# namada-net/masp

Hardware: AMD Instinct MI355X
Metric: Spend proofs/sec (higher is better)
Workload: dtype u32; 1 GPU; BASELINE.json configs[3]: batch of 256 distinct Spend proofs per step on one MI355X (throughput mode); proofs_per_gpu=4352, distinct_witnesses_per_gpu=256, ntt_log2=17, batch_cap=256, slots=4, calls_in_flight=4, hw_queues=4, parallelism=proofs sharded over 1 GPU(s), no data-path collective, gather of the proofs

## Files before the change

masp_amd/csrc/internal.h:

```cpp
#pragma once
#include <hip/hip_runtime.h>

#include <algorithm>
#include <array>
#include <condition_variable>
#include <cstring>
#include <deque>
#include <map>
#include <memory>
#include <mutex>
#include <shared_mutex>
#include <string>
#include <thread>
#include <vector>

#include "device/io.hpp"
#include "device/ntt_geom.h"
#include "launch.h"
#include "msm_host.h"
#include <atomic>
#include "util.h"

namespace masp {

template <class T>
struct DevBuf {
    T* p = nullptr;
    size_t cap = 0;
    ~DevBuf() { release(); }
    void release() {
        if (p) dev_free(p);
        p = nullptr;
        cap = 0;
    }
    int reserve(size_t n) {
        if (n <= cap) return MASP_HIP_OK;
        release();
        HIP_TRY(dev_malloc(&p, sizeof(T) * std::max<size_t>(n, 1)));
        cap = n;
        return MASP_HIP_OK;
    }
    int upload(const T* h, size_t n, hipStream_t s) {
        int rc = reserve(n);
        if (rc) return rc;
        if (n) HIP_TRY(hipMemcpyAsync(p, h, sizeof(T) * n, hipMemcpyHostToDevice, s));
        return MASP_HIP_OK;
    }
};

static inline Fr fr_from_u64_mont(uint64_t x) {
    Fr v = fe_zero<FrCfg>();
    v.v[0] = (uint32_t)x;
    v.v[1] = (uint32_t)(x >> 32);
    return fe_to_mont(v);
}
static inline Fr fr_const(const uint32_t* limbs) {
    Fr v;
    for (int i = 0; i < 8; ++i) v.v[i] = limbs[i];
    return v;
}

struct NttDomain {
    uint32_t logm = 0;
    size_t m = 0;
    DevBuf<Fr> tw_fwd, tw_inv, coset_scale, h_scale;
    Fr c_scale;
    int init(uint32_t logm_, hipStream_t s) {
        logm = logm_;
        m = (size_t)1 << logm;
        Fr omega = fr_const(FrCfg::ROOT_OF_UNITY);
        for (uint32_t i = logm; i < 32; ++i) omega = fe_sqr(omega);
        Fr omega_inv = fe_inv(omega);
        Fr minv = fe_inv(fr_from_u64_mont(m));
        Fr g = fr_const(FrCfg::GEN), ginv = fr_const(FrCfg::GEN_INV);
        uint32_t e[2] = {(uint32_t)m, (uint32_t)((uint64_t)m >> 32)};
        const Fr zinv = fe_inv(fe_sub(fe_pow(g, e, 2), fe_one<FrCfg>()));
        const Fr mzinv = fe_mul(minv, zinv);
        c_scale = fe_from_mont(mzinv);
        Fr one = fe_one<FrCfg>();
        size_t half = std::max<size_t>(m / 2, 1);
        int rc;
        if ((rc = tw_fwd.reserve(half)) || (rc = tw_inv.reserve(half)) || (rc = coset_scale.reserve(m)) || (rc = h_scale.reserve(m))) return rc;
        launch_fr_powers(s, tw_fwd.p, (uint32_t)half, omega, one, 0);
        launch_fr_powers(s, tw_inv.p, (uint32_t)half, omega_inv, one, 0);
        launch_fr_powers(s, coset_scale.p, (uint32_t)m, g, minv, 0);
        launch_fr_powers(s, h_scale.p, (uint32_t)m, ginv, mzinv, 1);
        HIP_TRY(hipStreamSynchronize(s));
        return MASP_HIP_OK;
    }
    void passes(hipStream_t s, Fr* data, const Fr* tw, uint32_t np = 1) const {
        for (uint32_t s0 = 0; s0 < logm;) {
            uint32_t nst = std::min<uint32_t>(NTT_LT, logm - s0);
            launch_ntt_pass(s, data, tw, logm, s0, nst, np);
            s0 += nst;
        }
    }
};

struct Circuit {
    uint32_t n_inputs = 0, n_aux = 0, n_constraints = 0, nrows = 0, logm = 0;
    size_t m = 0;
    DevBuf<uint32_t> rowptr[3], col[3];
    DevBuf<uint32_t> row_order[3];
    uint32_t n_long_rows[3] = {0, 0, 0};
    DevBuf<Fr> coef[3];
    DevBuf<uint32_t> a_var, b_var;
    uint32_t na = 0, nbq = 0;
    DevBuf<VkDevice> vk;
    DevBuf<G1Xyzz> fb1;
    DevBuf<G2Xyzz> fb2;
    BasesG1 h, l, a, b1;
    BasesG1 hl;
    BasesG2 b2;
    BasesG2 b2_lone;
    bool g1_endo = false;
    NttDomain* dom = nullptr;
};

struct Slot {
    hipStream_t stream = nullptr;
    hipEvent_t done = nullptr;
    MsmWorkspace<FpOps> ws1;
    MsmWorkspace<Fp2Ops> ws2;
    static constexpr int N_AUX = 4;
    hipStream_t aux[N_AUX] = {nullptr, nullptr, nullptr, nullptr};
    hipEvent_t ev_fork = nullptr, ev_sort_b = nullptr, ev_fixed = nullptr, ev_join[N_AUX] = {nullptr, nullptr, nullptr, nullptr};
    hipEvent_t ev_uploaded = nullptr;
    MsmWorkspace<FpOps> ws_l, ws_a, ws_b;
    DevBuf<Fr> w, inp, abc, wm, ev[3], x0, x1, h, hl, sa, sb;
    DevBuf<G1Xyzz> res1, asm1;
    DevBuf<G2Xyzz> res2, asm2;
    DevBuf<uint32_t> rs;
    DevBuf<uint8_t> proof;
    DevBuf<int> flags;
    MsmProfile prof;
    bool profiling = false;
    static constexpr int N_LONE_MARKS = 12;
    hipEvent_t ev_lone[N_LONE_MARKS] = {};
    bool lone_marked = false;
    void lone_mark(hipStream_t st, int id) {
        if (!profiling) return;
        if (!ev_lone[id] && hipEventCreate(&ev_lone[id]) != hipSuccess) return;
        (void)hipEventRecord(ev_lone[id], st);
        if (id == N_LONE_MARKS - 1) lone_marked = true;
    }
    uint32_t ntt_sub = 8;
    uint8_t* h_stage = nullptr;
    size_t h_stage_cap = 0;
    uint8_t* h_proof = nullptr;
    size_t h_proof_cap = 0;
    int* h_flags = nullptr;
    struct LoneGraph {
        const void *circuit, *w, *abc, *rs, *proof;
        size_t w_stride;
        uint32_t np;
        bool mont;
        int runs;
        bool dead;
        hipGraphExec_t exec;
    };
    std::vector<LoneGraph> graphs;
    uint64_t graph_epoch = 0;
    bool lone_graph = false;
    std::atomic<uint64_t> graph_launches{0};
    void drop_graphs() {
        for (auto& g : graphs)
            if (g.exec) hipGraphExecDestroy(g.exec);
        graphs.clear();
    }
    ~Slot() {
        drop_graphs();
        if (done) hipEventDestroy(done);
        for (hipEvent_t e : ev_join)
            if (e) hipEventDestroy(e);
        for (hipEvent_t e : ev_lone)
            if (e) hipEventDestroy(e);
        if (ev_fork) hipEventDestroy(ev_fork);
        if (ev_uploaded) hipEventDestroy(ev_uploaded);
        if (ev_sort_b) hipEventDestroy(ev_sort_b);
        if (ev_fixed) hipEventDestroy(ev_fixed);
        if (h_stage) hipHostFree(h_stage);
        if (h_proof) hipHostFree(h_proof);
        if (h_flags) hipHostFree(h_flags);
    }
    void configure(const masp_hip_options& o) {
        ntt_sub = (uint32_t)o.ntt_sub_batch;
        ws1.tree_levels = o.bucket_tree_levels;
        ws2.tree_levels = o.bucket_tree_levels_g2;
        ws1.tree_levels_shared = o.bucket_tree_levels_g2;
        ws1.tree_sub = ws2.tree_sub = (uint32_t)o.bucket_tree_sub_batch;
        ws2.tree.arena = &ws1.tree.own;
        ws1.tree.own.limit = (size_t)o.bucket_tree_scratch_mb << 20;
        lone_graph = o.lone_proof_graph > 0;
    }
    int init(const std::array<hipStream_t, 5>& streams) {
        stream = streams[0];
        for (int i = 0; i < N_AUX; ++i) aux[i] = streams[1 + i];
        HIP_TRY(hipEventCreateWithFlags(&done, hipEventDisableTiming));
        HIP_TRY(hipEventCreateWithFlags(&ev_fork, hipEventDisableTiming));
        HIP_TRY(hipEventCreateWithFlags(&ev_uploaded, hipEventDisableTiming));
        HIP_TRY(hipEventCreateWithFlags(&ev_sort_b, hipEventDisableTiming));
        HIP_TRY(hipEventCreateWithFlags(&ev_fixed, hipEventDisableTiming));
        for (hipEvent_t& e : ev_join) HIP_TRY(hipEventCreateWithFlags(&e, hipEventDisableTiming));
        HIP_TRY(hipHostMalloc(&h_flags, sizeof(int)));
        int rc;
        if ((rc = flags.reserve(1))) return rc;
        return reserve_batch(1);
    }
    int reserve_batch(size_t np) {
        int rc;
        if ((rc = res1.reserve(4 * np)) || (rc = res2.reserve(np)) || (rc = asm1.reserve(6 * np)) || (rc = asm2.reserve(np)) || (rc = rs.reserve(16 * np)) || (rc = proof.reserve(192 * np))) return rc;
        if (np > h_proof_cap) {
            if (h_proof) hipHostFree(h_proof);
            h_proof = nullptr;
            HIP_TRY(hipHostMalloc(&h_proof, 192 * np));
            h_proof_cap = np;
        }
        return MASP_HIP_OK;
    }
    int stage_reserve(size_t bytes) {
        if (bytes <= h_stage_cap) return MASP_HIP_OK;
        if (h_stage) hipHostFree(h_stage);
        h_stage = nullptr;
        HIP_TRY(hipHostMalloc(&h_stage, bytes));
        h_stage_cap = bytes;
        return MASP_HIP_OK;
    }
};

struct ResidentBatch {
    size_t n = 0;
    std::vector<uint32_t> circuit;
    std::vector<size_t> order;
    std::vector<size_t> w_off;
    DevBuf<Fr> w;
    DevBuf<uint32_t> rs;
};

struct StreamTable {
    hipStream_t main = nullptr;
    std::vector<std::array<hipStream_t, 5>> slot;
    hipStream_t vk[2] = {nullptr, nullptr};
    std::vector<hipStream_t> distinct() const {
        std::vector<hipStream_t> out;
        auto add = [&](hipStream_t s) {
            if (s && std::find(out.begin(), out.end(), s) == out.end()) out.push_back(s);
        };
        add(main);
        for (const auto& row : slot)
            for (hipStream_t s : row) add(s);
        for (hipStream_t s : vk) add(s);
        return out;
    }
    ~StreamTable() {
        for (hipStream_t s : distinct()) (void)hipStreamDestroy(s);
    }
};

}

using masp::Circuit;
using masp::DevBuf;
using masp::Fr;
using masp::G1Affine;
using masp::G1Xyzz;
using masp::G2Affine;
using masp::G2Xyzz;
using masp::NttDomain;
using masp::ResidentBatch;
using masp::Slot;

struct masp_hip_ctx {
    static constexpr size_t MAX_SLOTS = 64;
    int device = 0;
    std::vector<masp_hip_ctx*> children;
    masp_hip_options opt{};
    int n_slots = 4;
    size_t batch_cap = 256;
    std::shared_mutex mu;
    mutable std::mutex slot_mu;
    std::condition_variable slot_cv;
    std::vector<char> slot_busy;
    std::string err;
    masp::StreamTable streams;
    std::unique_ptr<Circuit> circ[MASP_HIP_MAX_CIRCUITS];
    std::map<uint32_t, std::unique_ptr<NttDomain>> domains;
    std::vector<std::unique_ptr<Slot>> slots;
    std::vector<std::unique_ptr<ResidentBatch>> batches;
    bool profiling = false;
    std::atomic<uint64_t> proofs_done{0};
    std::unique_ptr<std::atomic<int>[]> dev_status;
    std::atomic<uint64_t> requeued{0};
    std::atomic<uint32_t> fault_countdown{0};
    std::atomic<unsigned> vk_next{0};
    int main_streams_concurrent = 0;
    std::mutex upload_mu;
    hipEvent_t upload_tail = nullptr;
    std::atomic<uint64_t> block_tree_fallbacks{0};
    std::atomic<uint32_t> block_tree_sub{0xffffffffu};
    DevBuf<Fr> tmp_scalars;
    DevBuf<uint8_t> tmp_out;
    DevBuf<G1Xyzz> tmp_g1;
    DevBuf<G2Xyzz> tmp_g2;
    DevBuf<G1Affine> fb_g1;
    DevBuf<G2Affine> fb_g2;
    std::mutex jj_mu;
    DevBuf<uint8_t> jj_points, jj_scalars, jj_partial;
    DevBuf<int> jj_status;
    DevBuf<uint32_t> jj_out;
    struct NoteScanSet {
        DevBuf<uint8_t> epk, raw, ct, pts, status, hit_keys;
        DevBuf<uint32_t> count, hit_idx;
    };
    std::mutex ns_mu;
    NoteScanSet ns[2];
    DevBuf<uint32_t> ns_digits;
    std::atomic<int> ns_signed_digits{1}, ns_inversion{0};
    double ns_last_ms[2] = {0, 0};
};

namespace masp {

static inline int fail(masp_hip_ctx* ctx, int rc) {
    if (rc == MASP_HIP_E_HIP) {
        std::lock_guard<std::mutex> g(ctx->slot_mu);
        ctx->err = last_hip_error();
    }
    return rc;
}

#define FIRST_DEVICE(ctx) ((ctx) && !(ctx)->children.empty() ? (ctx)->children[0] : (ctx))

static inline int get_domain(masp_hip_ctx* ctx, uint32_t logm, NttDomain** out) {
    auto it = ctx->domains.find(logm);
    if (it == ctx->domains.end()) {
        std::unique_ptr<NttDomain> d(new NttDomain);
        int rc = d->init(logm, ctx->streams.main);
        if (rc) return rc;
        it = ctx->domains.emplace(logm, std::move(d)).first;
    }
    *out = it->second.get();
    return MASP_HIP_OK;
}

static inline uint32_t log2_ceil(uint32_t n) {
    uint32_t k = 0;
    while ((1ull << k) < n) ++k;
    return k;
}

}
```

masp_amd/csrc/prover.hip:

```cpp
#include <hip/hip_runtime.h>

#include <chrono>
#include <cstring>
#include <map>
#include <memory>
#include <algorithm>
#include <condition_variable>
#include <deque>
#include <mutex>
#include <shared_mutex>
#include <string>
#include <thread>
#include <vector>

#include "internal.h"

using namespace masp;

#ifndef MASP_UPLOAD_CHAIN
#define MASP_UPLOAD_CHAIN 1
#endif

namespace {

// ... 42 lines not shown
    ctx->slot_busy.push_back(busy);
    return MASP_HIP_OK;
}
static int ensure_slots(masp_hip_ctx* ctx, size_t want) {
    std::lock_guard<std::mutex> g(ctx->slot_mu);
    want = std::min(want, ctx->streams.slot.size());
    while (ctx->slots.size() < want)
        if (int rc = add_slot(ctx, 0)) return rc;
    for (auto& sl : ctx->slots) sl->profiling = ctx->profiling;
    return MASP_HIP_OK;
}
static int slot_try_acquire(masp_hip_ctx* ctx, size_t* si) {
    std::lock_guard<std::mutex> g(ctx->slot_mu);
    for (size_t i = 0; i < ctx->slots.size(); ++i)
        if (!ctx->slot_busy[i]) {
            ctx->slot_busy[i] = 1;
            *si = i;
            return MASP_HIP_OK;
        }
    if (ctx->slots.size() >= (size_t)ctx->n_slots) return -1;
    if (int rc = add_slot(ctx, 1)) return rc;
    *si = ctx->slots.size() - 1;
    return MASP_HIP_OK;
}
static size_t slot_acquire_blocking(masp_hip_ctx* ctx) {
    std::unique_lock<std::mutex> g(ctx->slot_mu);
    size_t found = 0;
    ctx->slot_cv.wait(g, [&] {
        for (size_t i = 0; i < ctx->slots.size(); ++i)
            if (!ctx->slot_busy[i]) {
                found = i;
                return true;
            }
        return false;
    });
    ctx->slot_busy[found] = 1;
    return found;
}
static void slot_release(masp_hip_ctx* ctx, size_t si) {
    bool idle = true;
    {
        std::lock_guard<std::mutex> g(ctx->slot_mu);
        ctx->slot_busy[si] = 0;
        for (char b : ctx->slot_busy) idle = idle && !b;
    }
    ctx->slot_cv.notify_one();
    if (idle) dev_free_drain();
}
static int enqueue_quotient(Slot& sl, const NttDomain& D, const Fr* const in[3], size_t in_stride, uint32_t nrows, bool mont_in, uint32_t np,
                            Fr* h_out = nullptr, size_t h_stride = 0) {
    hipStream_t s = sl.stream;
    const uint32_t m = (uint32_t)D.m, logm = D.logm;
    const uint32_t sub_max = sl.ntt_sub;
    const uint32_t sub = sub_max ? std::min(sub_max, np) : np;
    int rc;
    if ((rc = sl.x0.reserve((size_t)3 * m * sub)) || (rc = sl.x1.reserve((size_t)2 * m * sub))) return rc;
    if (!h_out) {
        if ((rc = sl.h.reserve((size_t)m * np))) return rc;
        h_out = sl.h.p;
        h_stride = m;
    }
    Fr *x0 = sl.x0.p, *x1 = sl.x1.p;
    for (uint32_t p0 = 0; p0 < np; p0 += sub) {
        const uint32_t q = std::min(sub, np - p0);
        const size_t part = (size_t)q * m;
        for (int i = 0; i < 3; ++i) {
            const Fr* src = in[i] + (size_t)p0 * in_stride;
            if (mont_in)
                launch_ntt_copy_bitrev(s, src, in_stride, nrows, x0 + i * part, logm, q);
            else
                launch_ntt_load_bitrev(s, src, in_stride, nrows, x0 + i * part, logm, q);
        }
        D.passes(s, x0, D.tw_inv.p, 3 * q);
        launch_ntt_scale_bitrev(s, x0, D.coset_scale.p, x1, logm, 2 * q);
        D.passes(s, x1, D.tw_fwd.p, 2 * q);
        launch_ntt_ab_bitrev(s, x1, x1 + part, x0, logm, q);
        D.passes(s, x0, D.tw_inv.p, q);
        launch_fr_scale_sub(s, x0, D.h_scale.p, x0 + 2 * part, D.c_scale, h_out + (size_t)p0 * h_stride, m, q, h_stride);
    }
    return MASP_HIP_OK;
}

static int enqueue_proofs(Slot& sl, Circuit& C, uint32_t np, const Fr* d_w, size_t w_stride, const Fr* const d_abc[3], const uint32_t* d_rs,
                          uint8_t* d_proof, bool aux_montgomery = false) {
    hipStream_t s = sl.stream;
    const uint32_t nv = C.n_inputs + C.n_aux;
    int rc;
    if ((rc = sl.reserve_batch(np))) return rc;
    if ((rc = sl.wm.reserve((size_t)nv * np))) return rc;
    const bool lone = np < 8;
    if (aux_montgomery) launch_fr_split_forms(s, const_cast<Fr*>(d_w), w_stride, sl.wm.p, nv, C.n_inputs, np, sl.flags.p);
    if (lone) {
        sl.lone_mark(s, 0);
        HIP_TRY(hipEventRecord(sl.ev_fork, s));
        for (int i = 0; i < Slot::N_AUX; ++i) HIP_TRY(hipStreamWaitEvent(sl.aux[i], sl.ev_fork, 0));
    }
    if (!aux_montgomery) launch_fr_to_mont(s, d_w, w_stride, sl.wm.p, nv, np, sl.flags.p);
    const Fr* in[3];
    bool mont_in;
    if (d_abc[0]) {
        in[0] = d_abc[0];
        in[1] = d_abc[1];
        in[2] = d_abc[2];
        mont_in = false;
    } else {
        R1csMatrices M;
        for (int i = 0; i < 3; ++i) {
            if ((rc = sl.ev[i].reserve((size_t)C.nrows * np))) return rc;
            M.rowptr[i] = C.rowptr[i].p;
            M.order[i] = C.row_order[i].p;
            M.n_long[i] = C.n_long_rows[i];
            M.col[i] = C.col[i].p;
            M.coef[i] = C.coef[i].p;
            M.out[i] = sl.ev[i].p;
            in[i] = sl.ev[i].p;
        }
        launch_r1cs_eval(s, M, sl.wm.p, nv, C.n_constraints, C.n_inputs, np);
        mont_in = true;
    }
    if ((rc = sl.sa.reserve((size_t)C.na * np)) || (rc = sl.sb.reserve((size_t)C.nbq * np))) return rc;
    MsmProfile* prof = sl.profiling ? &sl.prof : nullptr;
    const size_t m8 = C.m * 8;
    const bool share_b = C.nbq && C.b2.n == C.b1.n && C.b2.g.c == C.b1.g.c;
    if (lone) {
        launch_groth16_fixed_g1(sl.aux[0], C.fb1.p, d_rs, 16, sl.asm1.p, np);
        launch_groth16_fixed_g2(sl.aux[0], C.fb2.p, d_rs, 16, sl.asm2.p, np);
        HIP_TRY(hipEventRecord(sl.ev_fixed, sl.aux[0]));
        const bool own_b2 = C.b2_lone.n != 0;
        auto chain_a = [&]() -> int {
            int r;
            if (C.na) launch_gather_scalars(sl.aux[1], d_w, w_stride, C.a_var.p, C.na, sl.sa.p, np);
            if ((r = msm_enqueue(sl.aux[1], C.a, sl.ws_a, (const uint32_t*)sl.sa.p, (size_t)C.na * 8, sl.res1.p + 2, 4, np))) return r;
            sl.lone_mark(sl.aux[1], 1);
            launch_groth16_var_mul(sl.aux[1], 0, sl.res1.p, d_rs, 16, sl.asm1.p, np, C.g1_endo);
            sl.lone_mark(sl.aux[1], 2);
            return MASP_HIP_OK;
        };
        auto chain_b = [&]() -> int {
            int r;
            if (C.nbq) launch_gather_scalars(sl.aux[2], d_w, w_stride, C.b_var.p, C.nbq, sl.sb.p, np);
            HIP_TRY(hipEventRecord(sl.ev_sort_b, sl.aux[2]));
            if (share_b) {
                if ((r = msm_sort_enqueue(sl.aux[2], C.b1.n, C.b1.g, sl.ws_b.sort, (const uint32_t*)sl.sb.p, (size_t)C.nbq * 8, np))) return r;
                if (!own_b2) HIP_TRY(hipEventRecord(sl.ev_sort_b, sl.aux[2]));
                if ((r = msm_reduce_enqueue(sl.aux[2], C.b1, sl.ws_b.sort, sl.ws_b, sl.res1.p + 3, 4))) return r;
            } else if ((r = msm_enqueue(sl.aux[2], C.b1, sl.ws_b, (const uint32_t*)sl.sb.p, (size_t)C.nbq * 8, sl.res1.p + 3, 4, np))) {
                return r;
            }
            sl.lone_mark(sl.aux[2], 3);
            launch_groth16_var_mul(sl.aux[2], 1, sl.res1.p, d_rs, 16, sl.asm1.p, np, C.g1_endo);
            sl.lone_mark(sl.aux[2], 4);
            HIP_TRY(hipStreamWaitEvent(sl.aux[3], sl.ev_sort_b, 0));
            if (own_b2) {
                if ((r = msm_enqueue(sl.aux[3], C.b2_lone, sl.ws2, (const uint32_t*)sl.sb.p, (size_t)C.nbq * 8, sl.res2.p, 1, np))) return r;
            } else if (share_b) {
                if ((r = msm_reduce_enqueue(sl.aux[3], C.b2, sl.ws_b.sort, sl.ws2, sl.res2.p, 1))) return r;
            } else if ((r = msm_enqueue(sl.aux[3], C.b2, sl.ws2, (const uint32_t*)sl.sb.p, (size_t)C.nbq * 8, sl.res2.p, 1, np))) {
                return r;
            }
            sl.lone_mark(sl.aux[3], 5);
            HIP_TRY(hipStreamWaitEvent(sl.aux[3], sl.ev_fixed, 0));
            launch_groth16_finish_b(sl.aux[3], C.vk.p, sl.asm2.p, sl.res2.p, d_proof, np);
            sl.lone_mark(sl.aux[3], 6);
            return MASP_HIP_OK;
        };
        auto chain_l = [&]() -> int {
            return msm_enqueue(sl.aux[0], C.l, sl.ws_l, (const uint32_t*)(d_w + C.n_inputs), w_stride * 8, sl.res1.p + 1, 4, np);
        };
        if ((rc = chain_a()) || (rc = chain_b())) return rc;
        if ((rc = enqueue_quotient(sl, *C.dom, in, C.nrows, C.nrows, mont_in, np))) return rc;
        sl.lone_mark(s, 7);
        if ((rc = msm_enqueue(s, C.h, sl.ws1, (const uint32_t*)sl.h.p, m8, sl.res1.p + 0, 4, np, prof))) return rc;
        sl.lone_mark(s, 8);
        if ((rc = chain_l())) return rc;
        sl.lone_mark(sl.aux[0], 9);
        for (int i = 1; i < Slot::N_AUX - 1; ++i) {
            HIP_TRY(hipEventRecord(sl.ev_join[i], sl.aux[i]));
            HIP_TRY(hipStreamWaitEvent(sl.aux[0], sl.ev_join[i], 0));
        }
        launch_groth16_finish_ac_early(sl.aux[0], C.vk.p, sl.asm1.p, sl.res1.p, d_proof, np);
        HIP_TRY(hipEventRecord(sl.ev_join[0], sl.aux[0]));
        HIP_TRY(hipStreamWaitEvent(s, sl.ev_join[0], 0));
    } else {
        const size_t hl_stride = C.hl.n;
        if ((rc = sl.hl.reserve(hl_stride * np + 1))) return rc;
        if ((rc = enqueue_quotient(sl, *C.dom, in, C.nrows, C.nrows, mont_in, np, sl.hl.p, hl_stride))) return rc;
        HIP_TRY(hipMemcpy2DAsync(sl.hl.p + (C.m - 1), hl_stride * sizeof(Fr), d_w + C.n_inputs, w_stride * sizeof(Fr), (size_t)C.n_aux * sizeof(Fr), np,
                                 hipMemcpyDeviceToDevice, s));
        if (C.na) launch_gather_scalars(s, d_w, w_stride, C.a_var.p, C.na, sl.sa.p, np);
        if (C.nbq) launch_gather_scalars(s, d_w, w_stride, C.b_var.p, C.nbq, sl.sb.p, np);
        if ((rc = msm_enqueue(s, C.hl, sl.ws1, (const uint32_t*)sl.hl.p, hl_stride * 8, sl.res1.p + 0, 4, np, prof))) return rc;
        HIP_TRY(hipMemset2DAsync(sl.res1.p + 1, 4 * sizeof(G1Xyzz), 0, sizeof(G1Xyzz), np, s));
        const BasesG1 &Aq = C.a, &B1q = C.b1;
        const BasesG2& B2q = C.b2;
        const bool share_bq = share_b;
        if ((rc = msm_enqueue(s, Aq, sl.ws1, (const uint32_t*)sl.sa.p, (size_t)C.na * 8, sl.res1.p + 2, 4, np, prof))) return rc;
        if ((rc = msm_enqueue(s, B1q, sl.ws1, (const uint32_t*)sl.sb.p, (size_t)C.nbq * 8, sl.res1.p + 3, 4, np, prof))) return rc;
        if (share_bq) {
            if ((rc = msm_reduce_enqueue(s, B2q, sl.ws1.sort, sl.ws2, sl.res2.p, 1))) return rc;
        } else if ((rc = msm_enqueue(s, B2q, sl.ws2, (const uint32_t*)sl.sb.p, (size_t)C.nbq * 8, sl.res2.p, 1, np))) {
            return rc;
        }
    }
    if (!lone) {
        launch_groth16_fixed_g1(s, C.fb1.p, d_rs, 16, sl.asm1.p, np);
        launch_groth16_fixed_g2(s, C.fb2.p, d_rs, 16, sl.asm2.p, np);
                launch_groth16_var_mul(s, 2, sl.res1.p, d_rs, 16, sl.asm1.p, np, C.g1_endo);
        launch_groth16_finish_b(s, C.vk.p, sl.asm2.p, sl.res2.p, d_proof, np);
    }
    if (lone)
        launch_groth16_finish_c_late(s, sl.asm1.p, sl.res1.p, d_proof, np);
    else
        launch_groth16_finish_ac(s, C.vk.p, sl.asm1.p, sl.res1.p, d_proof, np);
    if (lone) {
        sl.lone_mark(s, 10);
        HIP_TRY(hipEventRecord(sl.ev_join[Slot::N_AUX - 1], sl.aux[Slot::N_AUX - 1]));
        HIP_TRY(hipStreamWaitEvent(s, sl.ev_join[Slot::N_AUX - 1], 0));
        sl.lone_mark(s, 11);
    }
    return MASP_HIP_OK;
}

static int enqueue_proofs_graphed(Slot& sl, Circuit& C, uint32_t np, const Fr* d_w, size_t w_stride, const Fr* const d_abc[3], const uint32_t* d_rs,
                                  uint8_t* d_proof, bool aux_montgomery) {
    if (np >= 8 || !sl.lone_graph || sl.profiling) return enqueue_proofs(sl, C, np, d_w, w_stride, d_abc, d_rs, d_proof, aux_montgomery);
    const uint64_t epoch = device_alloc_epoch().load(std::memory_order_relaxed);
    if (epoch != sl.graph_epoch) {
        sl.drop_graphs();
        sl.graph_epoch = epoch;
    }
    Slot::LoneGraph* e = nullptr;
    for (auto& g : sl.graphs)
        if (g.circuit == &C && g.np == np && g.w == d_w && g.w_stride == w_stride && g.abc == d_abc[0] && g.rs == d_rs && g.proof == d_proof &&
            g.mont == aux_montgomery)
            e = &g;
    if (!e) {
        if (sl.graphs.size() >= 16) sl.drop_graphs();
        sl.graphs.push_back(Slot::LoneGraph{&C, d_w, d_abc[0], d_rs, d_proof, w_stride, np, aux_montgomery, 0, false, nullptr});
        e = &sl.graphs.back();
    }
    if (e->exec) {
        HIP_TRY(hipGraphLaunch(e->exec, sl.stream));
        ++sl.graph_launches;
        return MASP_HIP_OK;
    }
    if (e->dead || e->runs == 0) {
        ++e->runs;
        return enqueue_proofs(sl, C, np, d_w, w_stride, d_abc, d_rs, d_proof, aux_montgomery);
    }
    bool ok = hipStreamBeginCapture(sl.stream, hipStreamCaptureModeThreadLocal) == hipSuccess;
    if (ok) {
        const int rc = enqueue_proofs(sl, C, np, d_w, w_stride, d_abc, d_rs, d_proof, aux_montgomery);
        hipGraph_t g = nullptr;
        const hipError_t ce = hipStreamEndCapture(sl.stream, &g);
        ok = rc == MASP_HIP_OK && ce == hipSuccess && g != nullptr && device_alloc_epoch().load(std::memory_order_relaxed) == epoch;
        if (ok) ok = hipGraphInstantiate(&e->exec, g, nullptr, nullptr, 0) == hipSuccess && e->exec != nullptr;
        if (g) hipGraphDestroy(g);
    }
    if (!ok) {
        (void)hipGetLastError();
        launch_error().clear();
        e->exec = nullptr;
        e->dead = true;
        sl.graph_epoch = device_alloc_epoch().load(std::memory_order_relaxed);
        return enqueue_proofs(sl, C, np, d_w, w_stride, d_abc, d_rs, d_proof, aux_montgomery);
    }
    HIP_TRY(hipGraphLaunch(e->exec, sl.stream));
    ++sl.graph_launches;
    return MASP_HIP_OK;
}

static bool rs_in_range(const uint8_t* x) {
    Fr v = fe_load_le<FrCfg>(x);
    return !fe_canonical_ge_mod(v);
}

struct ParamsLayout {
    const uint8_t *alpha_g1, *beta_g1, *beta_g2, *gamma_g2, *delta_g1, *delta_g2;
    const uint8_t *ic, *h, *l, *a, *b_g1, *b_g2;
    uint32_t n_ic, n_h, n_l, n_a, n_b1, n_b2;
};
static bool read_u32be(const uint8_t*& p, const uint8_t* end, uint32_t& v) {
    if (end - p < 4) return false;
    v = ((uint32_t)p[0] << 24) | ((uint32_t)p[1] << 16) | ((uint32_t)p[2] << 8) | p[3];
    p += 4;
    return true;
}
static bool parse_params(const uint8_t* buf, size_t len, ParamsLayout& L) {
    const uint8_t *p = buf, *end = buf + len;
    if (len < 864) return false;
    L.alpha_g1 = p; p += 96;
    L.beta_g1 = p;  p += 96;
    L.beta_g2 = p;  p += 192;
    L.gamma_g2 = p; p += 192;
    L.delta_g1 = p; p += 96;
    L.delta_g2 = p; p += 192;
    struct { const uint8_t** ptr; uint32_t* n; size_t sz; } secs[6] = {
        {&L.ic, &L.n_ic, 96}, {&L.h, &L.n_h, 96}, {&L.l, &L.n_l, 96}, {&L.a, &L.n_a, 96}, {&L.b_g1, &L.n_b1, 96}, {&L.b_g2, &L.n_b2, 192}};
    for (auto& sec : secs) {
        if (!read_u32be(p, end, *sec.n)) return false;
        if ((size_t)(end - p) < (size_t)*sec.n * sec.sz) return false;
        *sec.ptr = p;
        p += (size_t)*sec.n * sec.sz;
    }
    return true;
}

}
// ... 606 lines not shown
    return pending == 0 ? MASP_HIP_OK : MASP_HIP_E_HIP;
}

int masp_hip_prove_batch(masp_hip_ctx* ctx, size_t n, const masp_hip_job* jobs, uint8_t* proofs_out) {
    const ApiLaunchScope api_scope;
    if (!ctx || (n && (!jobs || !proofs_out))) return MASP_HIP_E_INVALID_ARG;
    if (!ctx->children.empty()) return prove_batch_multi(ctx, n, jobs, proofs_out);
    std::shared_lock<std::shared_mutex> lock(ctx->mu);
    if (int rc = validate_jobs(ctx, n, jobs)) return rc;
    for (uint32_t left = ctx->fault_countdown.load(); left != 0;) {
        if (!ctx->fault_countdown.compare_exchange_weak(left, left - 1)) continue;
        if (left == 1) {
            last_hip_error() = "injected fault (masp_hip_ctx_inject_fault): this device context's call fails as a lost GPU's would";
            return fail(ctx, MASP_HIP_E_HIP);
        }
        break;
    }
    hipSetDevice(ctx->device);
    struct Group {
        std::vector<size_t> idx;
    };
    std::vector<Group> groups;
    {
        std::map<std::pair<uint32_t, bool>, std::vector<size_t>> by_kind;
        for (size_t j = 0; j < n; ++j) by_kind[{jobs[j].circuit | (jobs[j].aux_form ? 0x100u : 0u), jobs[j].a != nullptr}].push_back(j);
        for (auto& kv : by_kind)
            for (auto& eg : even_groups(kv.second.size(), ctx->batch_cap)) {
                Group g;
                g.idx.assign(kv.second.begin() + eg.first, kv.second.begin() + eg.first + eg.second);
                groups.push_back(std::move(g));
            }
    }
    struct Owned {
        size_t si, gi;
    };
    std::deque<Owned> owned;
    int result = MASP_HIP_OK, rc;
    auto retire_oldest = [&]() -> size_t {
        Owned o = owned.front();
        owned.pop_front();
        Slot& sl = *ctx->slots[o.si];
        const Group& G = groups[o.gi];
        if (hipEventSynchronize(sl.done) != hipSuccess) {
            last_hip_error() = "event sync failed";
            result = fail(ctx, MASP_HIP_E_HIP);
        } else if (*sl.h_flags) {
            result = MASP_HIP_E_SCALAR_RANGE;
        } else if (result == MASP_HIP_OK) {
            for (size_t p = 0; p < G.idx.size(); ++p) memcpy(proofs_out + 192 * G.idx[p], sl.h_proof + 192 * p, 192);
        }
        return o.si;
    };
#ifdef MASP_ENQ_TIMING
    const auto tcall = std::chrono::steady_clock::now();
    auto ms_since = [&](std::chrono::steady_clock::time_point t0) { return std::chrono::duration<double, std::milli>(std::chrono::steady_clock::now() - t0).count(); };
#endif
    for (size_t gi = 0; gi < groups.size() && result == MASP_HIP_OK; ++gi) {
        size_t si = 0;
#ifdef MASP_ENQ_TIMING
        const auto tg0 = std::chrono::steady_clock::now();
#endif
        rc = slot_try_acquire(ctx, &si);
        if (rc > 0) {
            result = fail(ctx, rc);
            break;
        }
        if (rc < 0) si = owned.empty() ? slot_acquire_blocking(ctx) : retire_oldest();
        if (result) {
            slot_release(ctx, si);
            break;
        }
        const Group& G = groups[gi];
        Slot& sl = *ctx->slots[si];
        Circuit& C = *ctx->circ[jobs[G.idx[0]].circuit];
        const size_t nv = (size_t)C.n_inputs + C.n_aux, np = G.idx.size();
        const bool has_abc = jobs[G.idx[0]].a != nullptr;
#ifdef MASP_ENQ_TIMING
        const double t_wait = ms_since(tg0);
        const auto tg1 = std::chrono::steady_clock::now();
#endif
        const size_t w_bytes = 32 * nv * np, abc_bytes = has_abc ? 3 * 32 * (size_t)C.nrows * np : 0, rs_bytes = 64 * np;
        const size_t in_bytes = 32 * (size_t)C.n_inputs * np;
        bool ok = true;
        if ((rc = sl.stage_reserve(w_bytes + abc_bytes + rs_bytes + in_bytes)) || (rc = sl.w.reserve(nv * np)) || (rc = sl.inp.reserve((size_t)C.n_inputs * np)) ||
            (rc = sl.abc.reserve(has_abc ? 3 * (size_t)C.nrows * np : 1)) || (rc = sl.reserve_batch(np))) {
            result = fail(ctx, rc);
            ok = false;
        }
        if (ok) {
            uint8_t* hs = sl.h_stage;
            std::vector<char> direct(np, 0);
            bool any_staged = false;
            for (size_t p = 0; p < np; ++p) {
                hipPointerAttribute_t attr;
                direct[p] = hipPointerGetAttributes(&attr, jobs[G.idx[p]].aux) == hipSuccess && attr.type == hipMemoryTypeHost;
                any_staged = any_staged || !direct[p];
            }
            (void)hipGetLastError();
            for (size_t p = 0; p < np; ++p) {
                const masp_hip_job& J = jobs[G.idx[p]];
                memcpy(hs + 32 * nv * p, J.inputs, 32 * (size_t)C.n_inputs);
                memcpy(hs + w_bytes + abc_bytes + rs_bytes + 32 * (size_t)C.n_inputs * p, J.inputs, 32 * (size_t)C.n_inputs);
                if (!direct[p]) memcpy(hs + 32 * nv * p + 32 * (size_t)C.n_inputs, J.aux, 32 * (size_t)C.n_aux);
                if (has_abc) {
                    const uint8_t* src[3] = {J.a, J.b, J.c};
                    for (int i = 0; i < 3; ++i) memcpy(hs + w_bytes + 32 * (size_t)C.nrows * (np * i + p), src[i], 32 * (size_t)C.nrows);
                }
                memcpy(hs + w_bytes + abc_bytes + 64 * p, J.r, 32);
                memcpy(hs + w_bytes + abc_bytes + 64 * p + 32, J.s, 32);
            }
            hipStream_t s = sl.stream;
#if MASP_UPLOAD_CHAIN
            const bool chain = ctx->opt.lone_proof_graph == 0;
            std::unique_lock<std::mutex> upload_turn(ctx->upload_mu, std::defer_lock);
            if (chain) upload_turn.lock();
            if (chain && ctx->upload_tail && ctx->upload_tail != sl.ev_uploaded) ok = hipStreamWaitEvent(s, ctx->upload_tail, 0) == hipSuccess;
#endif
            if (!ok) {
            } else if (any_staged) {
                ok = hipMemcpyAsync(sl.w.p, hs, w_bytes, hipMemcpyHostToDevice, s) == hipSuccess;
            } else {
                ok = hipMemcpyAsync(sl.inp.p, hs + w_bytes + abc_bytes + rs_bytes, in_bytes, hipMemcpyHostToDevice, s) == hipSuccess &&
                     hipMemcpy2DAsync(sl.w.p, 32 * nv, sl.inp.p, 32 * (size_t)C.n_inputs, 32 * (size_t)C.n_inputs, np, hipMemcpyDeviceToDevice, s) ==
                         hipSuccess;
            }
            for (size_t p = 0; p < np && ok; ++p)
                if (direct[p])
                    ok = hipMemcpyAsync(sl.w.p + nv * p + C.n_inputs, jobs[G.idx[p]].aux, 32 * (size_t)C.n_aux, hipMemcpyHostToDevice, s) ==
                         hipSuccess;
            ok = ok && (!has_abc || hipMemcpyAsync(sl.abc.p, hs + w_bytes, abc_bytes, hipMemcpyHostToDevice, s) == hipSuccess) &&
                 hipMemcpyAsync(sl.rs.p, hs + w_bytes + abc_bytes, rs_bytes, hipMemcpyHostToDevice, s) == hipSuccess;
#if MASP_UPLOAD_CHAIN
            if (chain && ok && hipEventRecord(sl.ev_uploaded, s) == hipSuccess) ctx->upload_tail = sl.ev_uploaded;
#endif
            if (!ok) {
                last_hip_error() = std::string("H2D copy failed: ") + hipGetErrorString(hipGetLastError());
                result = fail(ctx, MASP_HIP_E_HIP);
            }
        }
        if (ok) {
            const Fr* abc[3] = {nullptr, nullptr, nullptr};
            if (has_abc)
                for (int i = 0; i < 3; ++i) abc[i] = sl.abc.p + (size_t)C.nrows * np * i;
            if (hipMemsetAsync(sl.flags.p, 0, sizeof(int), sl.stream) != hipSuccess) {
                last_hip_error() = "memset failed";
                result = fail(ctx, MASP_HIP_E_HIP);
                ok = false;
            } else {
#ifdef MASP_ENQ_TIMING
                const auto tq0 = std::chrono::steady_clock::now();
#endif
                if ((rc = enqueue_proofs_graphed(sl, C, (uint32_t)np, sl.w.p, nv, abc, sl.rs.p, sl.proof.p, jobs[G.idx[0]].aux_form == MASP_HIP_AUX_MONTGOMERY))) {
                    result = fail(ctx, rc);
                    ok = false;
                }
#ifdef MASP_ENQ_TIMING
                fprintf(stderr, "[enq] %zu proofs: %.3f ms\n", np, std::chrono::duration<double, std::milli>(std::chrono::steady_clock::now() - tq0).count());
#endif
            }
        }
        if (ok) {
            hipStream_t s = sl.stream;
            ok = hipMemcpyAsync(sl.h_proof, sl.proof.p, 192 * np, hipMemcpyDeviceToHost, s) == hipSuccess &&
                 hipMemcpyAsync(sl.h_flags, sl.flags.p, sizeof(int), hipMemcpyDeviceToHost, s) == hipSuccess &&
                 hipEventRecord(sl.done, s) == hipSuccess;
            if (!ok) {
                last_hip_error() = "D2H copy failed";
                result = fail(ctx, MASP_HIP_E_HIP);
            }
        }
        if (!ok) {
            for (int i = 0; i < Slot::N_AUX; ++i) hipStreamSynchronize(sl.aux[i]);
            hipStreamSynchronize(sl.stream);
            slot_release(ctx, si);
            break;
        }
        owned.push_back({si, gi});
#ifdef MASP_ENQ_TIMING
        fprintf(stderr, "[grp] call %p t=%8.2f ms group %zu circuit %u np %zu slot %zu: waited %.2f ms for the slot, staged + enqueued in %.2f ms\n", (void*)jobs,
                ms_since(tcall), gi, jobs[G.idx[0]].circuit, np, si, t_wait, ms_since(tg1));
#endif
    }
    while (!owned.empty()) slot_release(ctx, retire_oldest());
#ifdef MASP_ENQ_TIMING
    fprintf(stderr, "[call] %p done after %.2f ms (%zu jobs)\n", (void*)jobs, ms_since(tcall), n);
#endif
    if (result == MASP_HIP_OK) ctx->proofs_done += n;
    const int launch_rc = launch_status();
    if (launch_rc && result == MASP_HIP_OK) result = fail(ctx, launch_rc);
    if (hipGetLastError() != hipSuccess && result == MASP_HIP_OK) {
        last_hip_error() = "kernel launch failed";
        result = fail(ctx, MASP_HIP_E_HIP);
    }
    return result;
}

int masp_hip_prove(masp_hip_ctx* ctx, uint32_t slot, const uint8_t* inputs, const uint8_t* aux, const uint8_t* a, const uint8_t* b,
                   const uint8_t* c, const uint8_t r[32], const uint8_t s[32], uint8_t proof_out[192]) {
    if (!r || !s || !proof_out) return MASP_HIP_E_INVALID_ARG;
    masp_hip_job J;
    J.circuit = slot;
    J.inputs = inputs;
    J.aux = aux;
    J.a = a;
    J.b = b;
    J.c = c;
    J.aux_form = MASP_HIP_AUX_CANONICAL;
    J.reserved = 0;
    memcpy(J.r, r, 32);
    memcpy(J.s, s, 32);
    uint8_t tmp[192];
    int rc = masp_hip_prove_batch(ctx, 1, &J, tmp);
    if (rc == MASP_HIP_OK) memcpy(proof_out, tmp, 192);
    return rc;
}

}

template <class O, int BYTES>
static int msm_multi(masp_hip_ctx* ctx, const uint8_t* bases, size_t n, const uint8_t* scalars, size_t np, int window_bits, uint8_t* out) {
    if (!ctx || !out || !np || np > 256 || !n || !bases || !scalars || n > (1u << 22) || window_bits < 0 || window_bits == 1 || window_bits > 16)
        return MASP_HIP_E_INVALID_ARG;
    if (!ctx->children.empty()) ctx = ctx->children[0];
    std::unique_lock<std::shared_mutex> lock(ctx->mu);
    hipSetDevice(ctx->device);
    hipStream_t s = ctx->streams.main;
    for (size_t i = 0; i < n * np; ++i)
        if (!rs_in_range(scalars + 32 * i)) return MASP_HIP_E_SCALAR_RANGE;
    MsmBases<O, BYTES> B;
    MsmWorkspace<O> ws;
    ws.tree_levels = ctx->opt.bucket_tree_levels;
    ws.tree_sub = (uint32_t)ctx->opt.bucket_tree_sub_batch;
    ws.tree.own.limit = (size_t)ctx->opt.bucket_tree_scratch_mb << 20;
    struct Report {
        masp_hip_ctx* c;
        MsmWorkspace<O>& w;
        ~Report() {
            c->block_tree_fallbacks += w.tree_fallbacks;
            c->block_tree_sub = std::min<uint32_t>(c->block_tree_sub, w.tree_sub);
        }
    } report{ctx, ws};
    DevBuf<Xyzz<O>> res;
    DevBuf<uint8_t> d_out;
    int rc;
    if ((rc = B.load_host(bases, (uint32_t)n, s, 0xffffffffu, window_bits))) return fail(ctx, rc);
    if (B.import_status & (PT_BAD_FLAGS | PT_NOT_CANONICAL)) return MASP_HIP_E_PARAMS_FORMAT;
    if ((rc = ctx->tmp_scalars.upload((const Fr*)scalars, n * np, s)) || (rc = res.reserve(np)) || (rc = d_out.reserve(BYTES * np))) return fail(ctx, rc);
    if ((rc = msm_enqueue(s, B, ws, (const uint32_t*)ctx->tmp_scalars.p, n * 8, res.p, 1, (uint32_t)np))) return fail(ctx, rc);
    for (size_t p = 0; p < np; ++p) {
        if constexpr (BYTES == 96)
            launch_g1_export(s, res.p + p, d_out.p + BYTES * p);
        else
            launch_g2_export(s, res.p + p, d_out.p + BYTES * p);
    }
// ... 389 lines not shown
```

Before: 1393 proofs/s.

## Chunk witness upload and overlap per-chunk H2D with witness conversion and quotient NTT

Splits each batch's witness H2D upload into up to eight chunks aligned to the NTT sub-batch size. The uploads go on a shared main upload stream, and an event is recorded after each chunk. The slot stream waits on each chunk's event before running that chunk's Montgomery conversion, R1CS evaluation and quotient NTT, so compute on early proofs overlaps the transfer of later ones. Chunked uploads also skip waiting on a previous chunked upload tail, which adds event overhead, more small kernel launches and more complex cross-stream ordering.

```diff
diff --git a/masp_amd/csrc/internal.h b/masp_amd/csrc/internal.h
--- a/masp_amd/csrc/internal.h
+++ b/masp_amd/csrc/internal.h
@@ -18,6 +18,7 @@
 #include "device/ntt_geom.h"
 #include "launch.h"
 #include "msm_host.h"
+#include "upload_chunks.h"
 #include <atomic>
 #include "util.h"
 
@@ -126,6 +127,7 @@
     hipStream_t aux[N_AUX] = {nullptr, nullptr, nullptr, nullptr};
     hipEvent_t ev_fork = nullptr, ev_sort_b = nullptr, ev_fixed = nullptr, ev_join[N_AUX] = {nullptr, nullptr, nullptr, nullptr};
     hipEvent_t ev_uploaded = nullptr;
+    hipEvent_t ev_chunk[UPLOAD_MAX_CHUNKS] = {};
     MsmWorkspace<FpOps> ws_l, ws_a, ws_b;
     DevBuf<Fr> w, inp, abc, wm, ev[3], x0, x1, h, hl, sa, sb;
     DevBuf<G1Xyzz> res1, asm1;
@@ -177,6 +179,8 @@
             if (e) hipEventDestroy(e);
         if (ev_fork) hipEventDestroy(ev_fork);
         if (ev_uploaded) hipEventDestroy(ev_uploaded);
+        for (hipEvent_t e : ev_chunk)
+            if (e) hipEventDestroy(e);
         if (ev_sort_b) hipEventDestroy(ev_sort_b);
         if (ev_fixed) hipEventDestroy(ev_fixed);
         if (h_stage) hipHostFree(h_stage);
@@ -199,6 +203,7 @@
         HIP_TRY(hipEventCreateWithFlags(&done, hipEventDisableTiming));
         HIP_TRY(hipEventCreateWithFlags(&ev_fork, hipEventDisableTiming));
         HIP_TRY(hipEventCreateWithFlags(&ev_uploaded, hipEventDisableTiming));
+        for (hipEvent_t& e : ev_chunk) HIP_TRY(hipEventCreateWithFlags(&e, hipEventDisableTiming));
         HIP_TRY(hipEventCreateWithFlags(&ev_sort_b, hipEventDisableTiming));
         HIP_TRY(hipEventCreateWithFlags(&ev_fixed, hipEventDisableTiming));
         for (hipEvent_t& e : ev_join) HIP_TRY(hipEventCreateWithFlags(&e, hipEventDisableTiming));
@@ -296,6 +301,7 @@
     int main_streams_concurrent = 0;
     std::mutex upload_mu;
     hipEvent_t upload_tail = nullptr;
+    bool upload_tail_chunked = false;
     std::atomic<uint64_t> block_tree_fallbacks{0};
     std::atomic<uint32_t> block_tree_sub{0xffffffffu};
     DevBuf<Fr> tmp_scalars;
diff --git a/masp_amd/csrc/prover.hip b/masp_amd/csrc/prover.hip
--- a/masp_amd/csrc/prover.hip
+++ b/masp_amd/csrc/prover.hip
@@ -148,29 +148,38 @@
 }
 
 static int enqueue_proofs(Slot& sl, Circuit& C, uint32_t np, const Fr* d_w, size_t w_stride, const Fr* const d_abc[3], const uint32_t* d_rs,
-                          uint8_t* d_proof, bool aux_montgomery = false) {
+                          uint8_t* d_proof, bool aux_montgomery = false, const UploadPlan* up = nullptr) {
     hipStream_t s = sl.stream;
     const uint32_t nv = C.n_inputs + C.n_aux;
     int rc;
     if ((rc = sl.reserve_batch(np))) return rc;
     if ((rc = sl.wm.reserve((size_t)nv * np))) return rc;
-    const bool lone = np < 8;
-    if (aux_montgomery) launch_fr_split_forms(s, const_cast<Fr*>(d_w), w_stride, sl.wm.p, nv, C.n_inputs, np, sl.flags.p);
+    const bool lone = np < LONE_BATCH_BELOW;
+    const bool chunked = up && up->chunked() && !lone;
+    auto witness_forms = [&](uint32_t p0, uint32_t q) {
+        const Fr* w = d_w + (size_t)p0 * w_stride;
+        Fr* wm = sl.wm.p + (size_t)p0 * nv;
+        if (aux_montgomery)
+            launch_fr_split_forms(s, const_cast<Fr*>(w), w_stride, wm, nv, C.n_inputs, q, sl.flags.p);
+        else
+            launch_fr_to_mont(s, w, w_stride, wm, nv, q, sl.flags.p);
+    };
+    if (aux_montgomery && !chunked) witness_forms(0, np);
     if (lone) {
         sl.lone_mark(s, 0);
         HIP_TRY(hipEventRecord(sl.ev_fork, s));
         for (int i = 0; i < Slot::N_AUX; ++i) HIP_TRY(hipStreamWaitEvent(sl.aux[i], sl.ev_fork, 0));
     }
-    if (!aux_montgomery) launch_fr_to_mont(s, d_w, w_stride, sl.wm.p, nv, np, sl.flags.p);
+    if (!aux_montgomery && !chunked) witness_forms(0, np);
     const Fr* in[3];
     bool mont_in;
+    R1csMatrices M{};
     if (d_abc[0]) {
         in[0] = d_abc[0];
         in[1] = d_abc[1];
         in[2] = d_abc[2];
         mont_in = false;
     } else {
-        R1csMatrices M;
         for (int i = 0; i < 3; ++i) {
             if ((rc = sl.ev[i].reserve((size_t)C.nrows * np))) return rc;
             M.rowptr[i] = C.rowptr[i].p;
@@ -181,7 +190,7 @@
             M.out[i] = sl.ev[i].p;
             in[i] = sl.ev[i].p;
         }
-        launch_r1cs_eval(s, M, sl.wm.p, nv, C.n_constraints, C.n_inputs, np);
+        if (!chunked) launch_r1cs_eval(s, M, sl.wm.p, nv, C.n_constraints, C.n_inputs, np);
         mont_in = true;
     }
     if ((rc = sl.sa.reserve((size_t)C.na * np)) || (rc = sl.sb.reserve((size_t)C.nbq * np))) return rc;
@@ -250,7 +259,23 @@
     } else {
         const size_t hl_stride = C.hl.n;
         if ((rc = sl.hl.reserve(hl_stride * np + 1))) return rc;
-        if ((rc = enqueue_quotient(sl, *C.dom, in, C.nrows, C.nrows, mont_in, np, sl.hl.p, hl_stride))) return rc;
+        if (chunked) {
+            for (uint32_t c = 0; c < up->n; ++c) {
+                const uint32_t p0 = up->first(c), q = up->count(c);
+                HIP_TRY(hipStreamWaitEvent(s, sl.ev_chunk[c], 0));
+                witness_forms(p0, q);
+                const Fr* in_c[3];
+                R1csMatrices Mc = M;
+                for (int i = 0; i < 3; ++i) {
+                    in_c[i] = in[i] + (size_t)p0 * C.nrows;
+                    if (mont_in) Mc.out[i] = M.out[i] + (size_t)p0 * C.nrows;
+                }
+                if (mont_in) launch_r1cs_eval(s, Mc, sl.wm.p + (size_t)p0 * nv, nv, C.n_constraints, C.n_inputs, q);
+                if ((rc = enqueue_quotient(sl, *C.dom, in_c, C.nrows, C.nrows, mont_in, q, sl.hl.p + (size_t)p0 * hl_stride, hl_stride))) return rc;
+            }
+        } else if ((rc = enqueue_quotient(sl, *C.dom, in, C.nrows, C.nrows, mont_in, np, sl.hl.p, hl_stride))) {
+            return rc;
+        }
         HIP_TRY(hipMemcpy2DAsync(sl.hl.p + (C.m - 1), hl_stride * sizeof(Fr), d_w + C.n_inputs, w_stride * sizeof(Fr), (size_t)C.n_aux * sizeof(Fr), np,
                                  hipMemcpyDeviceToDevice, s));
         if (C.na) launch_gather_scalars(s, d_w, w_stride, C.a_var.p, C.na, sl.sa.p, np);
@@ -288,8 +313,8 @@
 }
 
 static int enqueue_proofs_graphed(Slot& sl, Circuit& C, uint32_t np, const Fr* d_w, size_t w_stride, const Fr* const d_abc[3], const uint32_t* d_rs,
-                                  uint8_t* d_proof, bool aux_montgomery) {
-    if (np >= 8 || !sl.lone_graph || sl.profiling) return enqueue_proofs(sl, C, np, d_w, w_stride, d_abc, d_rs, d_proof, aux_montgomery);
+                                  uint8_t* d_proof, bool aux_montgomery, const UploadPlan* up) {
+    if (np >= LONE_BATCH_BELOW || !sl.lone_graph || sl.profiling) return enqueue_proofs(sl, C, np, d_w, w_stride, d_abc, d_rs, d_proof, aux_montgomery, up);
     const uint64_t epoch = device_alloc_epoch().load(std::memory_order_relaxed);
     if (epoch != sl.graph_epoch) {
         sl.drop_graphs();
@@ -1062,6 +1087,8 @@
         const size_t w_bytes = 32 * nv * np, abc_bytes = has_abc ? 3 * 32 * (size_t)C.nrows * np : 0, rs_bytes = 64 * np;
         const size_t in_bytes = 32 * (size_t)C.n_inputs * np;
         bool ok = true;
+        UploadPlan plan;
+        hipStream_t upload_stream = nullptr;
         if ((rc = sl.stage_reserve(w_bytes + abc_bytes + rs_bytes + in_bytes)) || (rc = sl.w.reserve(nv * np)) || (rc = sl.inp.reserve((size_t)C.n_inputs * np)) ||
             (rc = sl.abc.reserve(has_abc ? 3 * (size_t)C.nrows * np : 1)) || (rc = sl.reserve_batch(np))) {
             result = fail(ctx, rc);
@@ -1089,29 +1116,45 @@
                 memcpy(hs + w_bytes + abc_bytes + 64 * p, J.r, 32);
                 memcpy(hs + w_bytes + abc_bytes + 64 * p + 32, J.s, 32);
             }
-            hipStream_t s = sl.stream;
+            plan = plan_upload_chunks((uint32_t)np, sl.ntt_sub);
+            if (ctx->opt.lone_proof_graph) plan.n = std::min(plan.n, 1u);
+            const bool chunked = plan.chunked();
+            hipStream_t s = chunked ? ctx->streams.main : sl.stream;
+            upload_stream = s;
 #if MASP_UPLOAD_CHAIN
             const bool chain = ctx->opt.lone_proof_graph == 0;
             std::unique_lock<std::mutex> upload_turn(ctx->upload_mu, std::defer_lock);
             if (chain) upload_turn.lock();
-            if (chain && ctx->upload_tail && ctx->upload_tail != sl.ev_uploaded) ok = hipStreamWaitEvent(s, ctx->upload_tail, 0) == hipSuccess;
+            if (chain && ctx->upload_tail && ctx->upload_tail != sl.ev_uploaded && !(chunked && ctx->upload_tail_chunked))
+                ok = hipStreamWaitEvent(s, ctx->upload_tail, 0) == hipSuccess;
+#else
+            std::unique_lock<std::mutex> upload_turn(ctx->upload_mu, std::defer_lock);
+            if (chunked) upload_turn.lock();
 #endif
-            if (!ok) {
-            } else if (any_staged) {
-                ok = hipMemcpyAsync(sl.w.p, hs, w_bytes, hipMemcpyHostToDevice, s) == hipSuccess;
-            } else {
+            ok = ok && hipMemcpyAsync(sl.rs.p, hs + w_bytes + abc_bytes, rs_bytes, hipMemcpyHostToDevice, s) == hipSuccess;
+            if (ok && !any_staged) {
                 ok = hipMemcpyAsync(sl.inp.p, hs + w_bytes + abc_bytes + rs_bytes, in_bytes, hipMemcpyHostToDevice, s) == hipSuccess &&
                      hipMemcpy2DAsync(sl.w.p, 32 * nv, sl.inp.p, 32 * (size_t)C.n_inputs, 32 * (size_t)C.n_inputs, np, hipMemcpyDeviceToDevice, s) ==
                          hipSuccess;
             }
-            for (size_t p = 0; p < np && ok; ++p)
-                if (direct[p])
-                    ok = hipMemcpyAsync(sl.w.p + nv * p + C.n_inputs, jobs[G.idx[p]].aux, 32 * (size_t)C.n_aux, hipMemcpyHostToDevice, s) ==
-                         hipSuccess;
-            ok = ok && (!has_abc || hipMemcpyAsync(sl.abc.p, hs + w_bytes, abc_bytes, hipMemcpyHostToDevice, s) == hipSuccess) &&
-                 hipMemcpyAsync(sl.rs.p, hs + w_bytes + abc_bytes, rs_bytes, hipMemcpyHostToDevice, s) == hipSuccess;
+            ok = ok && (!has_abc || hipMemcpyAsync(sl.abc.p, hs + w_bytes, abc_bytes, hipMemcpyHostToDevice, s) == hipSuccess);
+            for (uint32_t c = 0; c < plan.n && ok; ++c) {
+                const size_t p0 = plan.first(c), q = plan.count(c);
+                if (any_staged) ok = hipMemcpyAsync(sl.w.p + nv * p0, hs + 32 * nv * p0, 32 * nv * q, hipMemcpyHostToDevice, s) == hipSuccess;
+                for (size_t p = p0; p < p0 + q && ok; ++p)
+                    if (direct[p])
+                        ok = hipMemcpyAsync(sl.w.p + nv * p + C.n_inputs, jobs[G.idx[p]].aux, 32 * (size_t)C.n_aux, hipMemcpyHostToDevice, s) ==
+                             hipSuccess;
+                if (chunked) ok = ok && hipEventRecord(sl.ev_chunk[c], s) == hipSuccess;
+            }
 #if MASP_UPLOAD_CHAIN
-            if (chain && ok && hipEventRecord(sl.ev_uploaded, s) == hipSuccess) ctx->upload_tail = sl.ev_uploaded;
+            if (chain && ok) {
+                hipEvent_t tail = chunked ? sl.ev_chunk[plan.n - 1] : sl.ev_uploaded;
+                if (chunked || hipEventRecord(tail, s) == hipSuccess) {
+                    ctx->upload_tail = tail;
+                    ctx->upload_tail_chunked = chunked;
+                }
+            }
 #endif
             if (!ok) {
                 last_hip_error() = std::string("H2D copy failed: ") + hipGetErrorString(hipGetLastError());
@@ -1130,7 +1173,8 @@
 #ifdef MASP_ENQ_TIMING
                 const auto tq0 = std::chrono::steady_clock::now();
 #endif
-                if ((rc = enqueue_proofs_graphed(sl, C, (uint32_t)np, sl.w.p, nv, abc, sl.rs.p, sl.proof.p, jobs[G.idx[0]].aux_form == MASP_HIP_AUX_MONTGOMERY))) {
+                if ((rc = enqueue_proofs_graphed(sl, C, (uint32_t)np, sl.w.p, nv, abc, sl.rs.p, sl.proof.p, jobs[G.idx[0]].aux_form == MASP_HIP_AUX_MONTGOMERY,
+                                                 &plan))) {
                     result = fail(ctx, rc);
                     ok = false;
                 }
@@ -1150,6 +1194,7 @@
             }
         }
         if (!ok) {
+            if (upload_stream && upload_stream != sl.stream) hipStreamSynchronize(upload_stream);
             for (int i = 0; i < Slot::N_AUX; ++i) hipStreamSynchronize(sl.aux[i]);
             hipStreamSynchronize(sl.stream);
             slot_release(ctx, si);
diff --git a/masp_amd/csrc/upload_chunks.h b/masp_amd/csrc/upload_chunks.h
--- /dev/null
+++ b/masp_amd/csrc/upload_chunks.h
@@ -0,0 +1,34 @@
+#pragma once
+#include <algorithm>
+#include <cstdint>
+
+namespace masp {
+
+constexpr uint32_t UPLOAD_MAX_CHUNKS = 8;
+constexpr uint32_t LONE_BATCH_BELOW = 8;
+
+struct UploadPlan {
+    uint32_t np = 0;
+    uint32_t chunk = 0;
+    uint32_t n = 0;
+    bool chunked() const { return n >= 2; }
+    uint32_t first(uint32_t c) const { return c * chunk; }
+    uint32_t count(uint32_t c) const { return std::min(chunk, np - c * chunk); }
+    uint32_t chunk_of(uint32_t p) const { return p / chunk; }
+};
+
+static inline UploadPlan plan_upload_chunks(uint32_t np, uint32_t ntt_sub) {
+    UploadPlan P;
+    P.np = np;
+    P.chunk = np;
+    P.n = np ? 1 : 0;
+    if (np < LONE_BATCH_BELOW) return P;
+    const uint32_t sub = ntt_sub ? std::min(ntt_sub, np) : np;
+    const uint32_t n_sub = (np + sub - 1) / sub;
+    const uint32_t per = (n_sub + UPLOAD_MAX_CHUNKS - 1) / UPLOAD_MAX_CHUNKS;
+    P.chunk = sub * per;
+    P.n = (np + P.chunk - 1) / P.chunk;
+    return P;
+}
+
+}
```

Result: slower. 1363 proofs/s (-2.1%).
